# Shamir-Lab/Faucet

Measured on AMD Instinct MI355X. Metric: canonical k-mers/s (load+scan) at k=31, 100bp reads; % HBM roofline, higher is better.
Workload: dtype u64

## Files before the change

### faucet_amd/csrc/api.hip

```cpp
#include <cstdio>
#include <algorithm>
#include <string>

#include <chrono>
#include <thread>

#include "fgpu_ctx.h"

int fgpu_scan_export_impl(fgpu_ctx* ctx, void* dev_entries, uint64_t cap_entries, uint64_t* d_stamps, uint64_t* n_entries);
int fgpu_scan_import_impl(fgpu_ctx* ctx, const void* dev_entries, uint64_t n);
int fgpu_scan_download_impl(fgpu_ctx* ctx, uint64_t* keys_host, fgpu_junction* recs_host, uint64_t cap, uint64_t* n_out);

static thread_local std::string g_create_error;

int g_fgpu_trace = getenv("FGPU_TRACE") && getenv("FGPU_TRACE")[0] == '1';

int fgpu_ensure(fgpu_ctx* ctx, DevBuf* b, uint64_t bytes) {
    if (b->bytes >= bytes && b->p) return FGPU_OK;
    if (b->p) {
        FGPU_HIP(fgpu_sync_stream(ctx, ctx->stream));
        FGPU_HIP(hipFree(b->p));
        b->p = nullptr;
        b->bytes = 0;
    } else {
// ... 604 lines not shown
    if (nbytes) *nbytes = ctx->bloom_bytes;
    return FGPU_OK;
}

int fgpu_bitmap_or(fgpu_ctx* ctx, void* dst_dev, const void* src_dev, uint64_t nbytes) {
    if (!ctx || !dst_dev || !src_dev || (nbytes & 15)) return FGPU_ERR_ARG;
    return fgpu_util_or(ctx, dst_dev, src_dev, nbytes);
}

int fgpu_scan_resident_base(fgpu_ctx* ctx, uint64_t first_batch) {
    if (!ctx) return FGPU_ERR_ARG;
    if (ctx->phase != 0) { ctx->err = "scan_resident_base while a pass is open: between the load pass and fgpu_scan_begin"; return FGPU_ERR_STATE; }
    ctx->scan_resident_base = first_batch;
    return FGPU_OK;
}

int fgpu_scan_begin(fgpu_ctx* ctx) {
    if (!ctx) return FGPU_ERR_ARG;
    if (ctx->phase != 0) { ctx->err = "scan_begin while another pass is open"; return FGPU_ERR_STATE; }
    FGPU_HIP(hipSetDevice(ctx->prm.device));
    int rc = fgpu_bg_join(ctx);
    if (rc) return rc;
    if ((rc = fgpu_scan_alloc(ctx))) return rc;
    if ((rc = fgpu_scan_reset(ctx))) return rc;
    ctx->fixup_ready = false;
    FGPU_HIP(hipMemsetAsync(ctx->counters, 0, sizeof(DevCounters), ctx->stream));
    memset(&ctx->scan_stats, 0, sizeof(ctx->scan_stats));
    memset(ctx->counters_host, 0, sizeof(DevCounters));
    ctx->scan_windows = 0;
    ctx->scan_pieces_seen = 0;
    ctx->scan_piece_base = 0;
    ctx->scan_imported = 0;
    ctx->delta_next = 0;
    journal_recycle(ctx);
    ctx->journal_on = !(ctx->prm.flags & FGPU_FLAG_EAGER_FLAGS) && !ctx->eager_runtime;
    ctx->eager_scan = ctx->lazy_failed = ctx->capacity_failed = false;
    ctx->dl_keys_n = 0;
    ctx->late_acc[0] = ctx->late_acc[1] = ctx->late_acc[2] = 0;
    ctx->stops_delivered = 0;
    ctx->lp_applied_seq = 0;
    ctx->host_waits = 0;
    ctx->host_wait_ms = 0;
    ctx->wait_sites.clear();
    if (ctx->short_pf) FGPU_HIP(hipMemsetAsync(ctx->short_pf, 0, ctx->short_pf_tai / 8, ctx->stream));
    if ((rc = fgpu_long_pairs_reset(ctx))) return rc;
    ctx->have_import = false;
// ... 811 lines not shown
```

### faucet_amd/csrc/fgpu_ctx.h

```cpp
#pragma once
#include <chrono>
#include <hip/hip_runtime.h>
#include <stdint.h>
#include <stdio.h>
#include <string.h>

#include <string>
#include <thread>
#include <vector>

#include "../../include/faucet_gpu.h"
#include <deque>

#include "fgpu_device.h"

#define FGPU_PADW 8
#define FGPU_USUAL_SPAN (1ULL << 26)
#define FGPU_MAX_SPAN (1ULL << 26)

#define FGPU_RANGE_EVENTS 16
#define FGPU_RANGE_MIN (1ULL << 20)

struct DevBuf {
    void*    p = nullptr;
// ... 258 lines not shown
    uint32_t walk_heavy = 0;
    uint32_t* cl_members = nullptr;
    uint32_t* cl_roots = nullptr;
    void* wdesc = nullptr;
    uint64_t window_span = 1ULL << 17;
    uint64_t max_span = FGPU_MAX_SPAN;
    uint64_t settled_span = 0;
    uint64_t scan_piece_base = 0;
    uint64_t scan_imported = 0;
    bool hint_in_table = false;
    uint32_t hint_gen = 0;
    uint64_t hint_n = 0, hint_max_seq = 0;
    uint64_t hint_digest[2] = {0, 0};
    DevBuf delta_filter;
    uint64_t delta_filter_bits = 0;
    bool delta_ready = false;
    uint64_t delta_keys = 0;
    uint64_t refresh_full = 0, refresh_delta = 0, refresh_mismatch = 0;
    DevBuf cand_filter;
    uint64_t sparse_links = 0, full_links = 0;
    int dbg_stall_us = 0;
    bool dbg_delta_check = false;
    bool no_sparse_link = false;
    int scan_range_log2 = -1;
    DevBuf import_probe;
    uint64_t scan_grown = 0;

    DevCounters* counters = nullptr;
    DevCounters* counters_host = nullptr;

    fgpu_load_stats load_stats;
    uint64_t load_mark_hits = 0, load_mark_pending = 0;
    fgpu_scan_stats scan_stats;
    uint64_t scan_windows = 0;
    uint64_t scan_pieces_seen = 0;

    uint64_t adapt_followers = 0, adapt_pieces = 0;
    double host_ms[8] = {0, 0, 0, 0, 0, 0, 0, 0};
    bool repeats_seen_before = false;
    uint64_t calib_ovf = 0;
    uint64_t span_ceiling = ~0ULL;
    int adapt_vote = 0;
    uint64_t proven_span = 0;
    uint64_t adapt_overflows = 0;
    int calib_left = 0;
    uint64_t calib_f = 0, calib_p = 0;
// ... 154 lines not shown
int fgpu_resident_adopt(fgpu_ctx* ctx, const PackedBlock& b);
void fgpu_adopted_release(fgpu_ctx* ctx, std::vector<void*>* blocks);
int fgpu_stage_pack_keep(fgpu_ctx* ctx, const fgpu_reads* reads, uint64_t budget_left, PackedBlock* out, bool* no_memory);
void fgpu_estimate_drop_kept(fgpu_ctx* ctx);
int fgpu_load_sweep(fgpu_ctx* ctx);
int fgpu_stage_fixup(fgpu_ctx* ctx, const uint32_t* prefix);
int fgpu_stage_presence(fgpu_ctx* ctx);
int fgpu_epoch_before_batch(fgpu_ctx* ctx, uint64_t span);
int fgpu_epoch_after_batch(fgpu_ctx* ctx, uint64_t span);
enum { FGPU_TAKE_OK = 0, FGPU_TAKE_NO_BUDGET, FGPU_TAKE_NO_MEMORY };
int fgpu_resident_take(fgpu_ctx* ctx, const uint64_t (&parts)[5], bool budgeted, ResidentBatch** out, uint64_t* total);
int fgpu_pull_counters(fgpu_ctx* ctx);
int fgpu_check_reads(fgpu_ctx* ctx, const fgpu_reads* r);
void fgpu_load_pass_policy(fgpu_ctx* ctx);
int fgpu_load_pass_counters(fgpu_ctx* ctx);
int fgpu_load_pass_end(fgpu_ctx* ctx, fgpu_load_stats* stats);
int fgpu_load_pair_begin(fgpu_ctx* ctx);
int fgpu_load_pair_end(fgpu_ctx* ctx);
void fgpu_resident_reset(fgpu_ctx* ctx, bool keep_going);
int fgpu_stage_scan_pure(fgpu_ctx* ctx, uint64_t* n_pieces, bool one_range);
bool fgpu_walk_no_overlap();
int fgpu_stage_scan_walk(fgpu_ctx* ctx, uint64_t n_pieces);
int fgpu_stage_scan_need(fgpu_ctx* ctx);
int fgpu_stage_scan_need_lookup(fgpu_ctx* ctx, uint64_t w_lo, uint64_t w_hi);
int fgpu_stage_scan_need_prewalk(fgpu_ctx* ctx, uint64_t w_lo, uint64_t w_hi);
int fgpu_scan_refresh_planes(fgpu_ctx* ctx, BatchBufs* b);
int fgpu_scan_build_cand(fgpu_ctx* ctx, BatchBufs* b);
int fgpu_scan_import_probe(fgpu_ctx* ctx, const void* dev_entries, uint64_t n, uint64_t after_seq, uint32_t* dfilter, uint64_t dfilter_bits,
                           uint64_t* max_seq, uint64_t* n_newer, uint64_t digest[2]);
int fgpu_stage_scan_debug_drop(fgpu_ctx* ctx, uint64_t w_lo, uint64_t w_hi);
int fgpu_estimate_range_counts(fgpu_ctx* ctx, uint64_t g0, uint64_t g1, uint64_t h[2 * FGPU_EST_LEVELS + 1]);
void fgpu_estimate_close(fgpu_ctx* ctx, void** later);
int fgpu_estimate_finish(fgpu_ctx* ctx, fgpu_estimate* e, const char* who);
int fgpu_util_count_segments(fgpu_ctx* ctx, const void* bad, uint64_t n_words, int minlen);
int fgpu_util_popcount(fgpu_ctx* ctx, const void* dev, uint64_t nbytes, unsigned long long* dev_out);
int fgpu_util_or(fgpu_ctx* ctx, void* dst, const void* src, uint64_t nbytes);
int fgpu_util_probe_hash(fgpu_ctx* ctx, const uint64_t* d_kmers, uint64_t n, uint64_t* d_canon, uint64_t* d_hA, uint64_t* d_hB);
int fgpu_util_probe_contains(fgpu_ctx* ctx, const uint32_t* bloom, const uint64_t* d_canon, uint64_t n, unsigned char* d_out);
int fgpu_util_probe_stage3(fgpu_ctx* ctx, const uint64_t* d_kmers, uint64_t n, int mode, signed char* d_out);
int fgpu_scan_alloc(fgpu_ctx* ctx);
int fgpu_scan_harvest(fgpu_ctx* ctx, BatchBufs* b);
int fgpu_long_pairs_batch(fgpu_ctx* ctx, const fgpu_stop* d_stops, uint64_t n_stops, uint64_t n_reads);
int fgpu_long_pairs_reset(fgpu_ctx* ctx);
int fgpu_long_pairs_close(fgpu_ctx* ctx);
int fgpu_place_pair(fgpu_ctx* ctx);
int fgpu_scan_reset(fgpu_ctx* ctx);
// ... 6 lines not shown
```

### faucet_amd/csrc/scan_pure.hip

```cpp
#include <algorithm>

#include "fgpu_ctx.h"
#include "fgpu_flags.h"

namespace {

__global__ void __launch_bounds__(256) k_scan_same(const uint64_t* __restrict__ codes, const uint64_t* __restrict__ kept_codes, uint64_t n_code_words,
                                                   const uint64_t* __restrict__ bad, const uint64_t* __restrict__ kept_bad, uint64_t n_words,
                                                   uint32_t* same) {
    bool differ = false;
    for (uint64_t i = (uint64_t)blockIdx.x * blockDim.x + threadIdx.x; i < n_code_words; i += (uint64_t)gridDim.x * blockDim.x) {
        differ |= codes[i] != kept_codes[i];
        if (i < n_words) differ |= bad[i] != kept_bad[i];
    }
    if (__ballot(differ) && fd_lane() == 0) *same = 0;
}

__global__ void __launch_bounds__(256) k_scan_valid(const uint64_t* __restrict__ codes, const uint64_t* __restrict__ bad,
                                                    uint64_t T, uint64_t n_words, FdParams fp, const uint32_t* __restrict__ bloom,
                                                    const uint64_t* __restrict__ sure, const uint32_t* __restrict__ same,
                                                    uint64_t* __restrict__ valid, DevCounters* cnt) {
    unsigned long long n_ok = 0, n_reused = 0;
    const uint64_t total = n_words * 64;
    const bool reuse = sure && *same != 0;
    for (uint64_t p = (uint64_t)blockIdx.x * blockDim.x + threadIdx.x; p < total; p += (uint64_t)gridDim.x * blockDim.x) {
        bool ok = p < T && fd_window_ok(bad, p, fp.k);
        bool v = false;
        if (ok) {
            n_ok++;
            if (reuse && ((sure[p >> 6] >> (p & 63)) & 1ULL)) {
                v = true;
                n_reused++;
            } else {
                v = fd_bloom_contains_canon(bloom, fd_canon(fd_kmer_at(codes, p, fp.k), fp.k), fp.tai_mask, fp.n_hash);
            }
        }
        uint64_t vm = __ballot(v);
        if (fd_lane() == 0) valid[p >> 6] = vm;
    }
    block_add(&cnt->kmers, n_ok);
    block_add(&cnt->valid_reused, n_reused);
}

__global__ void __launch_bounds__(256) k_scan_pieces(const uint64_t* __restrict__ valid, const uint64_t* __restrict__ bad,
                                                     uint64_t n_words, FdParams fp, int check_segment,
                                                     unsigned long long* pm, uint64_t* __restrict__ ps, DevCounters* cnt) {
    unsigned long long n_pieces = 0;
    for (uint64_t w = (uint64_t)blockIdx.x * blockDim.x + threadIdx.x; w < n_words; w += (uint64_t)gridDim.x * blockDim.x) {
        uint64_t vw = valid[w];
        uint64_t prev = w ? valid[w - 1] >> 63 : 0;
        uint64_t starts = vw & ~((vw << 1) | prev);
        uint64_t psw = 0;
        while (starts) {
            const int sbit = __builtin_ctzll(starts);
            starts &= starts - 1;
            const uint64_t p = w * 64 + sbit;
            uint64_t q = p, len = 0;
            for (;;) {
                uint64_t bits = ~fd_bits_at(valid, q);
                if (bits) { len += __builtin_ctzll(bits); break; }
                len += 64;
                q += 64;
            }
            bool piece = len >= (uint64_t)fp.k;
            if (piece && check_segment) {
                uint64_t b = p;
                while (b > 0 && !((bad[(b - 1) >> 6] >> ((b - 1) & 63)) & 1ULL)) b--;
                uint64_t e = p;
                for (;;) {
                    uint64_t bits = fd_bits_at(bad, e);
                    if (bits) { e += __builtin_ctzll(bits); break; }
// ... 443 lines not shown
    int rc;
    uint64_t first, further;
    scan_range_plan(ctx, bb, one_range, &first, &further);
    const uint64_t first_words = std::max<uint64_t>(first / 64, 1), further_words = std::max<uint64_t>(further / 64, 1);
    const uint64_t reach_words = (bb.max_piece_span + 63) / 64 + 1;
    bb.range_first = first_words * 64;
    bb.range_span = further_words * 64;
    bb.n_ranges = bb.n_words <= first_words ? 1 : 1 + (bb.n_words - first_words + further_words - 1) / further_words;
    uint64_t looked = 0;
    for (uint64_t r = 0, lo = 0; lo < bb.n_words; r++) {
        const uint64_t hi = std::min(bb.n_words, lo + (r ? further_words : first_words));
        const uint64_t look_to = std::min(bb.n_words, hi + reach_words);
        if (looked < look_to) {
            if ((rc = fgpu_stage_scan_need_lookup(ctx, looked, look_to))) return rc;
            looked = look_to;
        }
        if ((rc = fgpu_stage_scan_need_prewalk(ctx, lo, hi)) || (rc = scan_pure_flags(ctx, lo, hi)) || (rc = fgpu_stage_scan_debug_drop(ctx, lo, hi))) return rc;
        if (bb.n_ranges > 1) FGPU_HIP(hipEventRecord(bb.range_ev[r % FGPU_RANGE_EVENTS], ctx->stream));
        lo = hi;
    }
    return FGPU_OK;
}

int fgpu_stage_scan_pure(fgpu_ctx* ctx, uint64_t* n_pieces, bool one_range) {
    BatchBufs& bb = *ctx->cur;
    *n_pieces = 0;
    bb.n_pieces = 0;
    bb.n_ranges = 0;
    if (bb.T == 0) return FGPU_OK;
    const uint64_t wb = (bb.n_words + FGPU_PADW) * 8;
    int rc;
    DevBuf* planes[] = {&bb.valid, &bb.pm, &bb.ps, &bb.ff, &bb.fb, &bb.cf0, &bb.cf1, &bb.cb0, &bb.cb1, &bb.inF, &bb.inB, &bb.lk, &bb.nF, &bb.nB, &bb.need};
    for (DevBuf* b : planes)
        if ((rc = fgpu_ensure_b(ctx, b, wb))) return rc;
    if ((rc = fgpu_ensure_b(ctx, &bb.ps_prefix, (bb.n_words + FGPU_PADW + bb.n_words / SCAN_BLOCK + 2) * 4))) return rc;
    const double t_a = fgpu_host_now();
    FGPU_HIP(hipMemsetAsync(bb.valid.p, 0, wb, ctx->stream));
    FGPU_HIP(hipMemsetAsync(bb.pm.p, 0, wb, ctx->stream));
    FGPU_HIP(hipMemsetAsync(bb.ps.p, 0, wb, ctx->stream));

    const unsigned grid = fgpu_grid(bb.n_words * 64, 256);
    const unsigned wgrid = fgpu_grid(bb.n_words, 256);
    if ((rc = fgpu_util_count_segments(ctx, ctx->cur->bad.p, ctx->cur->n_words, ctx->fd.k + 2 * ctx->fd.j + 1))) return rc;
    const uint64_t kept_index = ctx->scan_resident_base + ctx->scan_batch_index;
    const ResidentBatch* kept = kept_index < ctx->resident_count ? ctx->resident[kept_index] : nullptr;
    ctx->scan_batch_index++;
    if (kept && (kept->T != bb.T || kept->n_words != bb.n_words)) kept = nullptr;
    if (kept) {
        if ((rc = fgpu_ensure_b(ctx, &bb.same, 64))) return rc;
        FGPU_HIP(hipMemsetAsync(bb.same.p, 0x01, 4, ctx->stream));
        const uint64_t ncw = 2 * bb.n_words;
        FGPU_LAUNCH("scan_same", k_scan_same, fgpu_grid(ncw, 256), 256, (const uint64_t*)bb.codes.p, (const uint64_t*)kept->codes_p(), ncw,
                    (const uint64_t*)bb.bad.p, (const uint64_t*)kept->bad_p(), bb.n_words, (uint32_t*)bb.same.p);
    }
    FGPU_LAUNCH("scan_valid", k_scan_valid, grid, 256, (const uint64_t*)bb.codes.p, (const uint64_t*)bb.bad.p, bb.T, bb.n_words, ctx->fd,
                (const uint32_t*)ctx->bloo2, kept ? (const uint64_t*)kept->sure.p : (const uint64_t*)nullptr,
                kept ? (const uint32_t*)bb.same.p : (const uint32_t*)nullptr, (uint64_t*)bb.valid.p, ctx->counters);
    const int check_segment = ctx->fd.k < 2 * ctx->fd.j + 2;
    FGPU_LAUNCH("scan_pieces", k_scan_pieces, wgrid, 256, (const uint64_t*)bb.valid.p, (const uint64_t*)bb.bad.p, bb.n_words, ctx->fd,
                check_segment, (unsigned long long*)bb.pm.p, (uint64_t*)bb.ps.p, ctx->counters);
    uint32_t* prefix = (uint32_t*)bb.ps_prefix.p;
    uint32_t* block_sums = prefix + bb.n_words + FGPU_PADW;
    const uint32_t nblk = fgpu_blocks(bb.n_words + 1, SCAN_BLOCK);
    const uint64_t nw1 = bb.n_words + 1;
    FGPU_LAUNCH("prefix_block", k_prefix_block, nblk, SCAN_BLOCK, (const uint64_t*)bb.ps.p, nw1, prefix, block_sums);
    FGPU_LAUNCH("prefix_sums", k_prefix_sums, 1, SCAN_BLOCK, block_sums, nblk);
    FGPU_LAUNCH("prefix_apply", k_prefix_apply, fgpu_blocks(nw1, 256), 256, prefix, (const uint32_t*)block_sums, nw1);
    FGPU_HIP(hipMemcpyAsync(ctx->counters_host, ctx->counters, sizeof(DevCounters), hipMemcpyDeviceToHost, ctx->stream));
    const double t_b = fgpu_host_now();
    FGPU_HIP(fgpu_sync_stream(ctx, ctx->stream));
    const double t_c = fgpu_host_now();
    ctx->host_ms[2] += t_b - t_a;
    ctx->host_ms[3] += t_c - t_b;
    bb.max_piece_span = ctx->counters_host->max_read_len + 64;
    const uint64_t np = ctx->counters_host->pieces - ctx->scan_pieces_seen;
    ctx->scan_pieces_seen = ctx->counters_host->pieces;
    *n_pieces = np;
    bb.n_pieces = np;
    if ((rc = fgpu_ensure_b(ctx, &bb.pieces, (np + 1) * sizeof(uint2)))) return rc;
    if (np) {
        FGPU_LAUNCH("piece_list", k_scan_piece_list, wgrid, 256, (const uint64_t*)bb.ps.p, (const uint64_t*)bb.pm.p,
                    (const uint32_t*)prefix, bb.n_words, (uint2*)bb.pieces.p);
        if (ctx->record_stops) {
            if ((rc = fgpu_ensure_b(ctx, &bb.piece_read, np * 4))) return rc;
            FGPU_LAUNCH("piece_read", k_scan_piece_read, fgpu_blocks(np, 256), 256, (const uint2*)bb.pieces.p, np, bb.d_offs, bb.n_reads,
                        (uint32_t*)bb.piece_read.p);
        }
        if ((rc = fgpu_stage_scan_need(ctx))) return rc;
        DevBuf* outs[] = {&bb.ff, &bb.fb, &bb.cf0, &bb.cf1, &bb.cb0, &bb.cb1};
        for (DevBuf* o : outs) FGPU_HIP(hipMemsetAsync(o->p, 0, wb, ctx->stream));
        if ((rc = scan_pure_back(ctx, one_range))) return rc;
    }
    ctx->host_ms[4] += fgpu_host_now() - t_c;
    return FGPU_OK;
}
```

### faucet_amd/csrc/scan_table.hip

```cpp
#include <algorithm>

#include "walk_tables.h"

#include <rocprim/rocprim.hpp>

namespace {

__global__ void __launch_bounds__(256) k_export(JTable jt, FdParams fp, ExportEntry* out, uint64_t* stamps_out, unsigned long long* n_out) {
    __shared__ unsigned wave_total[4];
    __shared__ unsigned long long block_base;
    const uint64_t n_slots = jt.mask + 1;
    const uint64_t per_block = ((n_slots + gridDim.x - 1) / gridDim.x + 255) & ~255ULL;
    const uint64_t lo = (uint64_t)blockIdx.x * per_block;
    const uint64_t hi = lo + per_block < n_slots ? lo + per_block : n_slots;
    const int wave = (int)(threadIdx.x >> 6);
    unsigned long long mine = 0;
    for (uint64_t s = lo + threadIdx.x; s < hi; s += 256) {
        const uint64_t w = jt.keys[s];
        if (w != J_EMPTY) mine += ((w >> 62) & 1ULL) + ((w >> 63) & 1ULL);
    }
    for (int o = 32; o > 0; o >>= 1) mine += __shfl_down(mine, o, 64);
    if (fd_lane() == 0) wave_total[wave] = (unsigned)mine;
    __syncthreads();
    if (threadIdx.x == 0) {
// ... 141 lines not shown
}

int fgpu_scan_import_probe(fgpu_ctx* ctx, const void* dev_entries, uint64_t n, uint64_t after_seq, uint32_t* dfilter, uint64_t dfilter_bits,
                           uint64_t* max_seq, uint64_t* n_newer, uint64_t digest[2]) {
    *max_seq = *n_newer = 0;
    digest[0] = digest[1] = 0;
    if (!n) return FGPU_OK;
    if (int rc = fgpu_ensure(ctx, &ctx->import_probe, 32)) return rc;
    FGPU_HIP(hipMemsetAsync(ctx->import_probe.p, 0, 32, ctx->stream));
    FGPU_LAUNCH("import", k_import_probe, (unsigned)std::min<uint64_t>(fgpu_blocks(n, 256), 4096), 256, (const ExportEntry*)dev_entries, n, ctx->fd, after_seq, dfilter,
                dfilter_bits ? dfilter_bits - 1 : 0, (unsigned long long*)ctx->import_probe.p);
    unsigned long long out[4] = {0, 0, 0, 0};
    FGPU_HIP(hipMemcpyAsync(out, ctx->import_probe.p, 32, hipMemcpyDeviceToHost, ctx->stream));
    FGPU_HIP(fgpu_sync_stream(ctx, ctx->stream));
    *max_seq = out[0];
    *n_newer = out[1];
    digest[0] = out[2];
    digest[1] = out[3];
    return FGPU_OK;
}

int fgpu_scan_clear_table(fgpu_ctx* ctx) {
    FGPU_HIP(hipMemsetAsync(ctx->jkeys, 0xFF, ctx->jcap * 8, ctx->stream));
    FGPU_HIP(hipMemsetAsync(ctx->jrecs, 0, ctx->jcap * 32, ctx->stream));
    FGPU_HIP(hipMemsetAsync(ctx->jfilter, 0, ctx->jcap * 2 / 8, ctx->stream));
    return FGPU_OK;
}

static int jt_replace_arrays(fgpu_ctx* ctx, uint64_t new_cap, const char* no_memory) {
    uint64_t* nk = nullptr; uint8_t* nr = nullptr; uint64_t* ns = nullptr; uint32_t* nf = nullptr;
    if (hipMalloc(&nk, new_cap * 8) != hipSuccess || hipMalloc(&nr, new_cap * 32) != hipSuccess || hipMalloc(&ns, new_cap * 16) != hipSuccess ||
        hipMalloc(&nf, new_cap * 2 / 8) != hipSuccess) {
        (void)hipGetLastError();
        hipFree(nk); hipFree(nr); hipFree(ns); hipFree(nf);
        ctx->err = no_memory + std::to_string(new_cap) + " slots";
        return FGPU_ERR_NOMEM;
    }
    hipFree(ctx->jkeys); hipFree(ctx->jrecs); hipFree(ctx->jstamps); hipFree(ctx->jfilter);
    ctx->jkeys = nk; ctx->jrecs = nr; ctx->jstamps = ns; ctx->jfilter = nf;
    ctx->jcap = new_cap;
    return FGPU_OK;
}

int fgpu_scan_grow(fgpu_ctx* ctx, uint64_t new_cap) {
    if (new_cap <= ctx->jcap) return FGPU_OK;
    if (ctx->wstream) FGPU_HIP(fgpu_sync_stream(ctx, ctx->wstream));
    FGPU_HIP(fgpu_sync_stream(ctx, ctx->stream));
    FGPU_HIP(hipMemcpyAsync(&ctx->counters_host->n_junctions, &ctx->counters->n_junctions, 8, hipMemcpyDeviceToHost, ctx->stream));
// ... 110 lines not shown
```

### faucet_amd/csrc/scan_walk.hip

```cpp
#include <cstring>
#include <algorithm>

#include "fgpu_flags.h"
#include "walk_tables.h"

namespace {

__device__ __forceinline__ uint32_t uf_find(uint32_t* parent, uint32_t x) {
    uint32_t p = ld_agent(&parent[x]);
    while (p != x) {
        uint32_t gp = ld_agent(&parent[p]);
        if (gp != p) atomicMin(&parent[x], gp);
        x = p;
        p = gp;
    }
    return x;
}

__device__ __forceinline__ void uf_union(uint32_t* parent, uint32_t a, uint32_t b) {
    for (;;) {
        a = uf_find(parent, a);
        b = uf_find(parent, b);
        if (a == b) return;
        if (a < b) { uint32_t t = a; a = b; b = t; }
// ... 639 lines not shown
        KO_T0();
        out.addr = (uint64_t*)(wc.jt.recs + (known_slot * 2 + orient) * 16);
        out.lo = ld_agent(&out.addr[0]);
        out.hi = ld_agent(&out.addr[1]);
        wc.created_now = false;
        if (out.lo == 0xFFFFFFFFFFFFFFF1ULL) return false;
        KO_T1(wc.cnt, 3);
        return true;
    }
    const uint64_t home = fd_mix(canon) & wc.jt.mask;
    const uint64_t* spec = (const uint64_t*)(wc.jt.recs + (home * 2 + orient) * 16);
    const uint64_t w_first = ld_agent(&wc.jt.keys[home]);
    const uint64_t spec_lo = MODE == WALK_KO ? ld_agent(&spec[0]) : spec[0], spec_hi = MODE == WALK_KO ? ld_agent(&spec[1]) : spec[1];
    if (!jt_find_or_claim(wc.jt, canon, home, w_first, slot, present, wc.cnt)) {
        atomicOr(&wc.cnt->error_flags, 1ULL);
        return false;
    }
    out.addr = (uint64_t*)(wc.jt.recs + (slot * 2 + orient) * 16);
    wc.created_now = false;
    if (!((present >> orient) & 1u)) {
        wc.created_now = true;
        atomicOr(&wc.pl.cr[pos >> 6], 1ULL << (pos & 63));
        out.lo = out.hi = 0;
        if (MODE == WALK_KO) st_agent(&wc.jt.stamps[slot * 2 + orient], stamp);
        else wc.jt.stamps[slot * 2 + orient] = stamp;
        atomicOr((unsigned long long*)&wc.jt.keys[slot], 1ULL << (62 + orient));
        const uint64_t hb = jt_filter_bit(wc.jt, canon);
        atomicOr(&wc.jt.filter[hb >> 5], 1u << (hb & 31));
        wc.n_created++;
    } else if (slot == home) {
        out.lo = spec_lo;
        out.hi = spec_hi;
    } else {
        out.lo = MODE == WALK_KO ? ld_agent(&out.addr[0]) : out.addr[0];
        out.hi = MODE == WALK_KO ? ld_agent(&out.addr[1]) : out.addr[1];
    }
    return true;
}


__device__ __forceinline__ bool junction_find(const WalkCtx& wc, uint64_t key, RecRegs& out) {
    const uint64_t rc = fd_revcomp(key, wc.fp.k);
    const uint64_t canon = key < rc ? key : rc;
    const int orient = key == canon ? 0 : 1;
    uint64_t slot;
    uint32_t present;
// ... 893 lines not shown
    const uint4 r = ovw_live_bits(wc.pl.codes, wc.fp.k, v.p0 + 64 * c, where, wc.jt.keys, wc.jt.mask, ow.have_prev ? &ow.prev : nullptr, ow.time);
    mF = (uint64_t)r.x | ((uint64_t)r.y << 32);
    mB = (uint64_t)r.z | ((uint64_t)r.w << 32);
}
__device__ __forceinline__ void ovw_mark_created(const WalkCtx& wc, PieceView& v, uint64_t key) {
    const int k = wc.fp.k;
    for (uint32_t c = 0; c < 2; c++) {
        uint64_t w = c == 0 ? v.lk0 : v.lk1;
        while (w) {
            const uint32_t b = (uint32_t)__builtin_ctzll(w);
            w &= w - 1;
            const uint64_t km = pv_kmer(v, wc.pl.codes, v.p0 + 64 * c + b, k);
            if (km == key) { if (c == 0) v.xF0 |= 1ULL << b; else v.xF1 |= 1ULL << b; }
            if (fd_revcomp(km, k) == key) { if (c == 0) v.xB0 |= 1ULL << b; else v.xB1 |= 1ULL << b; }
        }
    }
}

struct OvwRec {
    uint32_t rec;
    uint64_t lo;
    bool present;
};
__device__ __forceinline__ bool ovw_record(WalkCtx& wc, uint64_t key, OvwRec& out) {
    const uint64_t rc = fd_revcomp(key, wc.fp.k);
    const uint64_t canon = key < rc ? key : rc;
    const int orient = key == canon ? 0 : 1;
    const uint64_t home = fd_mix(canon) & wc.jt.mask;
    const uint64_t* spec = (const uint64_t*)(wc.jt.recs + (home * 2 + orient) * 16);
    const uint64_t w_first = ld_agent(&wc.jt.keys[home]);
    const uint64_t spec_lo = spec[0];
    uint64_t slot;
    uint32_t present;
    if (!jt_find_or_claim(wc.jt, canon, home, w_first, slot, present, wc.cnt)) return false;
    out.rec = (uint32_t)(slot * 2 + orient);
    out.present = (present >> orient) & 1u;
    out.lo = !out.present ? 0ULL : slot == home ? spec_lo : ((const uint64_t*)(wc.jt.recs + (slot * 2 + orient) * 16))[0];
    return true;
}

__device__ __forceinline__ void ovw_walk_piece(WalkCtx& wc, OvwWalk& ow, uint64_t p0, uint32_t nwin) {
    const int k = wc.fp.k, j = wc.fp.j;
    const int tmax = 2 * (int)nwin - 2 - 2 * j;
    const int spacer = 2 * wc.fp.max_spacer - 1;
    PieceView v;
    pv_load(v, wc.pl, p0, nwin);
// ... 70 lines not shown
        const int ext_fwd = fwd ? real : 4, ext_bwd = fwd ? 4 : real;
        OvwRec r;
        {
            const uint32_t at = ow.n_new + (have_last ? 1u : 0u);
            const uint4 o = ow.have_old && at < ow.n_old ? ow.log[at] : make_uint4(0, 0xFFFFFFFFu, 0, 0);
            if ((o.y & 0xFFFF) == (uint32_t)tn && !((o.y >> 16) & OVW_F_FAKE)) {
                r.rec = o.x;
                r.present = ((o.y >> 16) & OVW_F_PRESENT) != 0;
                r.lo = (uint64_t)o.w | ((uint64_t)((o.z >> 8) & 0xFF) << 32);
            } else if (!ovw_record(wc, key, r)) { wc.fail = 1; return; }
        }
        const bool revisit = ovw_seen_test_and_set(r.rec);
        last_pos = tn;
        const uint32_t d_in = (uint32_t)((have_last ? tn - last_t : tn - 2 * j) & 0xFF);
        if (have_last) {
            pend.y |= (OVW_F_LINK_F | OVW_F_DF) << 16;
            pend.z = (pend.z & ~0xFFu) | d_in;
            if (d_in > ((last_lo >> (8 * last_ext_fwd)) & 0xFF) && !ovw_post(ow.cur, pend.x, (uint32_t)last_ext_fwd, ow.time, d_in)) { wc.fail = 1; return; }
            ovw_emit(ow, pend);
        }
        const bool created = !r.present && !(ow.have_prev && ovw_before(ow.prev, r.rec, OVW_CREATION, ow.time)) && !(revisit && ovw_own_created(ow, r.rec));
        uint32_t flags = (created ? OVW_F_CREATED : 0u) | ((uint32_t)real << 1) | (have_last ? OVW_F_LINK_B : 0u) | (r.present ? OVW_F_PRESENT : 0u);
        pend = ovw_pack(r.rec, (uint32_t)tn, flags, d_in, 0, r.lo);
        if (created && !ovw_post(ow.cur, r.rec, OVW_CREATION, ow.time, 1)) { wc.fail = 1; return; }
        if (d_in > ((r.lo >> (8 * ext_bwd)) & 0xFF) && !ovw_post(ow.cur, r.rec, (uint32_t)ext_bwd, ow.time, d_in)) { wc.fail = 1; return; }
        if (created) ovw_mark_created(wc, v, key);
        uint32_t d = (uint32_t)((r.lo >> (8 * ext_fwd)) & 0xFF);
        if (ow.have_prev) d = max(d, ovw_before(ow.prev, r.rec, (uint32_t)ext_fwd, ow.time));
        if (revisit) d = max(d, ovw_own(ow, r.rec, (uint32_t)ext_fwd, pend, true));
        have_last = true;
        last_lo = r.lo;
        last_t = tn;
        last_ext_fwd = ext_fwd;
        if (d < 1) d = 1;
        t = tn + (int)d;
        wc.nb_processed += 1;
        wc.nb_skipped += (unsigned long long)(d - 1);
        if (ow.overflow) { wc.fail = 1; return; }
    }

    if (!have_last) {
        wc.nb_no_juncs++;
        const int len = (int)nwin + k - 1;
        const int m = len / 2 - k / 2;
        const uint64_t key = pv_kmer(v, wc.pl.codes, p0 + m, k);
        const int real = pv_base(v, wc.pl.codes, p0 + m + k);
        const int tm = 2 * m + 1;
        OvwRec r;
        if (!ovw_record(wc, key, r)) { wc.fail = 1; return; }
        const bool created = !r.present && !(ow.have_prev && ovw_before(ow.prev, r.rec, OVW_CREATION, ow.time));
        const uint32_t d_b = (uint32_t)((tm - 2 * j) & 0xFF), d_f = (uint32_t)(((2 * (int)nwin - 1 - tm) - 2 * j) & 0xFF);
        if (created && !ovw_post(ow.cur, r.rec, OVW_CREATION, ow.time, 1)) { wc.fail = 1; return; }
        if (d_b > ((r.lo >> 32) & 0xFF) && !ovw_post(ow.cur, r.rec, 4u, ow.time, d_b)) { wc.fail = 1; return; }
        if (d_f > ((r.lo >> (8 * real)) & 0xFF) && !ovw_post(ow.cur, r.rec, (uint32_t)real, ow.time, d_f)) { wc.fail = 1; return; }
        uint4 e = ovw_pack(r.rec, (uint32_t)tm, (created ? OVW_F_CREATED : 0u) | ((uint32_t)real << 1) | OVW_F_FAKE | OVW_F_DF | (r.present ? OVW_F_PRESENT : 0u), d_b, d_f, r.lo);
        ovw_emit(ow, e);
    } else {
        const uint32_t d_f = (uint32_t)(((2 * (int)nwin - 1 - last_t) - 2 * j) & 0xFF);
        pend.y |= OVW_F_DF << 16;
        pend.z = (pend.z & ~0xFFu) | d_f;
        if (d_f > ((last_lo >> (8 * last_ext_fwd)) & 0xFF) && !ovw_post(ow.cur, pend.x, (uint32_t)last_ext_fwd, ow.time, d_f)) { wc.fail = 1; return; }
        ovw_emit(ow, pend);
    }
    if (ow.overflow) wc.fail = 1;
    if (ow.have_old)
        for (uint32_t i = ow.n_new; i < ow.n_old; i++) {
            const uint4 o = ow.log[i];
            if (ovw_event_sig(o)) ovw_mark(ow, o);
        }
}

__global__ void __launch_bounds__(256) k_ovw_reset(uint32_t* state, uint32_t* filt, uint32_t filt_words3, uint32_t* longp, uint32_t n_pieces,
                                                   uint32_t* marks, uint32_t mark_words3) {
    const uint32_t i = blockIdx.x * blockDim.x + threadIdx.x, stride = gridDim.x * blockDim.x;
// ... 481 lines not shown
            return FGPU_ERR_NOMEM;
        }
        ctx->max_span >>= 1;
    }
}

int fgpu_scan_reset(fgpu_ctx* ctx) {
    if (int rc = fgpu_scan_clear_table(ctx)) return rc;
    if (!ctx->wt_epoch) FGPU_HIP(hipMemsetAsync(ctx->wkeys, 0, ctx->wcap * 8, ctx->stream));
    FGPU_HIP(hipMemsetAsync(ctx->wbits, 0, 2 * (1ULL << ctx->wbits_log2) / 8, ctx->stream));
    FGPU_LAUNCH("iota", k_iota_u32, 64, 256, ctx->uf_parent, (uint64_t)ctx->wmax);
    FGPU_LAUNCH("iota", k_iota_u32, 64, 256, ctx->uf_parent + ctx->wmax, (uint64_t)ctx->wmax);
    FGPU_HIP(hipMemsetAsync(ctx->cl_count, 0, 2 * ctx->wmax * 4, ctx->stream));
    FGPU_HIP(hipMemsetAsync(ctx->cl_offset, 0xFF, 2 * ctx->wmax * 4, ctx->stream));
    FGPU_HIP(hipMemsetAsync(ctx->cl_fail, 0, 2 * ctx->wmax * 4, ctx->stream));
    FGPU_HIP(hipMemsetAsync(ctx->ko_hk, 0xFF, (size_t)ctx->ko_hk_cap * 4 * 2, ctx->stream));
    FGPU_HIP(hipMemsetAsync(ctx->ko_hk + 2 * (size_t)ctx->ko_hk_cap, 0, (size_t)ctx->ko_hk_cap * 4, ctx->stream));
    FGPU_HIP(hipMemsetAsync(ctx->ko_piece, 0, (size_t)ctx->wmax * 4 * 2 + 64, ctx->stream));
    return FGPU_OK;
}

int fgpu_stage_scan_need(fgpu_ctx* ctx) {
    BatchBufs& bb = *ctx->cur;
    const uint64_t wb = (bb.n_words + FGPU_PADW) * 8;
    const bool eager = (ctx->prm.flags & FGPU_FLAG_EAGER_FLAGS) || ctx->eager_runtime || ctx->eager_scan;
    FGPU_HIP(hipMemsetAsync(bb.need.p, eager ? 0xFF : 0, wb, ctx->stream));
    if (!bb.n_pieces) return FGPU_OK;
    return fgpu_ensure_b(ctx, &bb.kh, (bb.n_words + FGPU_PADW) * 64 * 4);
}

int fgpu_stage_scan_need_lookup(fgpu_ctx* ctx, uint64_t w_lo, uint64_t w_hi) {
    BatchBufs& bb = *ctx->cur;
    if (!bb.n_pieces || w_lo >= w_hi) return FGPU_OK;
    FGPU_LAUNCH("need_lookup", k_need_lookup, fgpu_grid((w_hi - w_lo) * 64, 256), 256, (const uint64_t*)bb.codes.p, (const uint64_t*)bb.pm.p,
                w_hi, ctx->fd, make_jt(ctx), (uint64_t*)bb.nF.p, (uint64_t*)bb.nB.p, (uint32_t*)bb.kh.p, w_lo);
    return FGPU_OK;
}

int fgpu_stage_scan_need_prewalk(fgpu_ctx* ctx, uint64_t w_lo, uint64_t w_hi) {
    BatchBufs& bb = *ctx->cur;
    const bool eager = (ctx->prm.flags & FGPU_FLAG_EAGER_FLAGS) || ctx->eager_runtime || ctx->eager_scan;
    if (eager || !bb.n_pieces || w_lo >= w_hi) return FGPU_OK;
    static const int need_tight = getenv("FGPU_NEED_TIGHT") ? atoi(getenv("FGPU_NEED_TIGHT")) : 2;
    const uint64_t most = std::min<uint64_t>(bb.n_pieces, (w_hi - w_lo) * 64 / (uint64_t)(ctx->fd.k + 1) + 2);
    FGPU_LAUNCH("need_prewalk", k_need_prewalk, fgpu_grid(most, 256), 256, (const uint64_t*)bb.codes.p, (const uint2*)bb.pieces.p,
                (const uint32_t*)bb.ps_prefix.p, w_lo, w_hi, ctx->fd, make_jt(ctx), (const uint64_t*)bb.nF.p, (const uint64_t*)bb.nB.p,
                (unsigned long long*)bb.need.p, need_tight);
    return FGPU_OK;
}

int fgpu_scan_refresh_planes(fgpu_ctx* ctx, BatchBufs* b) {
    if (!b->n_pieces || !b->T) return FGPU_OK;
    JTable jt = make_jt(ctx);
    ctx->launch_stream = ctx->stream;
    FGPU_LAUNCH("need_lookup", k_refresh_lookup, fgpu_grid(b->n_words * 64, 256), 256, (const uint64_t*)b->codes.p, (const uint64_t*)b->pm.p, b->n_words,
                ctx->fd, jt, (const uint32_t*)jt.filter, jt.filter_mask, (uint64_t*)b->nF.p, (uint64_t*)b->nB.p, (const uint32_t*)b->kh.p, 0, (uint64_t*)nullptr);
    if (b->pure_done) FGPU_HIP(hipEventRecord(b->pure_done, ctx->stream));
    return FGPU_OK;
}

int fgpu_scan_build_cand(fgpu_ctx* ctx, BatchBufs* b) {
    b->cand_gen = 0;
    if (!b->n_pieces || !b->T) return FGPU_OK;
    int rc;
    const uint64_t wb = (b->n_words + FGPU_PADW) * 8;
    if ((rc = fgpu_ensure_b(ctx, &b->cand, wb)) || (rc = fgpu_ensure(ctx, &ctx->cand_filter, (1ULL << CAND_FILTER_LOG2) / 8))) return rc;
    ctx->launch_stream = ctx->stream;
    FGPU_HIP(hipMemsetAsync(ctx->cand_filter.p, 0, (1ULL << CAND_FILTER_LOG2) / 8, ctx->stream));
    FGPU_HIP(hipMemsetAsync(b->cand.p, 0, wb, ctx->stream));
    const unsigned word_blocks = std::min(fgpu_blocks(b->n_words, 256), 2048u), piece_blocks = std::min(fgpu_blocks(b->n_pieces, 256), 2048u);
    FGPU_LAUNCH("cand_plane", k_cand_mark, word_blocks + piece_blocks, 256, (const uint64_t*)b->pm.p, (const uint64_t*)b->nF.p, (const uint64_t*)b->nB.p,
                (const uint64_t*)b->ff.p, (const uint64_t*)b->fb.p, (const uint32_t*)b->kh.p, b->n_words, (const uint2*)b->pieces.p, b->n_pieces, ctx->fd,
                (uint32_t*)ctx->cand_filter.p, word_blocks);
    FGPU_LAUNCH("cand_plane", k_cand_probe, fgpu_grid(b->n_words * 64, 256), 256, (const uint64_t*)b->pm.p, (const uint32_t*)b->kh.p, b->n_words,
                (const uint32_t*)ctx->cand_filter.p, (uint64_t*)b->cand.p);
    if (b->pure_done) FGPU_HIP(hipEventRecord(b->pure_done, ctx->stream));
    b->cand_gen = ctx->hint_gen;
    return FGPU_OK;
}

int fgpu_stage_scan_debug_drop(fgpu_ctx* ctx, uint64_t w_lo, uint64_t w_hi) {
    static const int drop = getenv("FGPU_DEBUG_NEED_DROP") ? atoi(getenv("FGPU_DEBUG_NEED_DROP")) : 0;
    BatchBufs& bb = *ctx->cur;
    if (!drop || !bb.n_pieces || w_lo >= w_hi) return FGPU_OK;
    if (drop == 2 && ((ctx->prm.flags & FGPU_FLAG_EAGER_FLAGS) || ctx->eager_runtime || ctx->eager_scan)) return FGPU_OK;
    FGPU_LAUNCH("debug_need_drop", k_debug_need_drop, fgpu_grid(w_hi - w_lo, 256), 256, w_lo, w_hi, (uint64_t*)bb.ff.p, (uint64_t*)bb.fb.p,
                (uint64_t*)bb.need.p, (uint64_t*)bb.cf0.p, (uint64_t*)bb.cf1.p, (uint64_t*)bb.cb0.p, (uint64_t*)bb.cb1.p, drop,
                (const uint64_t*)bb.pm.p, (const uint32_t*)bb.kh.p);
    return FGPU_OK;
}

static int env_int(const char* name, int absent) { const char* e = getenv(name); return e ? atoi(e) : absent; }
static bool env_is_one(const char* name) { const char* e = getenv(name); return e && e[0] == '1'; }
struct WalkKnobs {
    const int dbg_walk = env_int("FGPU_DEBUG_WALK", 0);
    const bool serial_clean = env_is_one("FGPU_SERIAL_CLEAN");
    const bool no_overlap = env_is_one("FGPU_NO_OVERLAP");
    const bool no_whole_batch = getenv("FGPU_NO_WHOLE_BATCH") != nullptr;
    const unsigned cluster_grid = (unsigned)std::max(1, env_int("FGPU_CLUSTER_GRID", 256));
    const uint64_t refresh_div = (uint64_t)std::max(1, env_int("FGPU_REFRESH_DIV", 4));
    const unsigned delta_per_block = (unsigned)std::max(1, env_int("FGPU_DELTA_PER_BLOCK", 1024));
    const int ko_avg = getenv("FGPU_WALK_KO_AVG") ? std::min(255, std::max(0, env_int("FGPU_WALK_KO_AVG", 0))) : -1;
    const int ko_avg_min = getenv("FGPU_WALK_KO_AVG_MIN") ? std::min(255, std::max(1, env_int("FGPU_WALK_KO_AVG_MIN", 0))) : -1;
    const uint32_t ko_ticket = (uint32_t)std::max(64, env_int("FGPU_KO_TICKET", 64) / 64 * 64);
    const int ovw_followers = env_int("FGPU_OVW_FOLLOWERS", 0);
    const bool ovw_beside = !env_is_one("FGPU_OVW_SERIAL");
    const unsigned walk_dyn_grid = (unsigned)std::max(1, env_int("FGPU_WALK_DYN_GRID", 1024));
    const bool dbg_span = getenv("FGPU_DEBUG_SPAN") != nullptr;
// ... 458 lines not shown
```

Baseline: 6.037 billion.

## Fold scan plane memsets into scan kernels and drop junction record clearing

```diff
diff --git a/faucet_amd/csrc/api.hip b/faucet_amd/csrc/api.hip
--- a/faucet_amd/csrc/api.hip
+++ b/faucet_amd/csrc/api.hip
@@ -650,6 +650,7 @@
     int rc = fgpu_bg_join(ctx);
     if (rc) return rc;
     if ((rc = fgpu_scan_alloc(ctx))) return rc;
+    ctx->debug_poison = getenv("FGPU_DEBUG_POISON") && getenv("FGPU_DEBUG_POISON")[0] == '1';
     if ((rc = fgpu_scan_reset(ctx))) return rc;
     ctx->fixup_ready = false;
     FGPU_HIP(hipMemsetAsync(ctx->counters, 0, sizeof(DevCounters), ctx->stream));
diff --git a/faucet_amd/csrc/fgpu_ctx.h b/faucet_amd/csrc/fgpu_ctx.h
--- a/faucet_amd/csrc/fgpu_ctx.h
+++ b/faucet_amd/csrc/fgpu_ctx.h
@@ -304,6 +304,7 @@
     int dbg_stall_us = 0;
     bool dbg_delta_check = false;
     bool no_sparse_link = false;
+    bool debug_poison = false;
     int scan_range_log2 = -1;
     DevBuf import_probe;
     uint64_t scan_grown = 0;
@@ -504,6 +505,7 @@
 bool fgpu_walk_no_overlap();
 int fgpu_stage_scan_walk(fgpu_ctx* ctx, uint64_t n_pieces);
 int fgpu_stage_scan_need(fgpu_ctx* ctx);
+static inline bool fgpu_scan_eager(const fgpu_ctx* ctx) { return (ctx->prm.flags & FGPU_FLAG_EAGER_FLAGS) || ctx->eager_runtime || ctx->eager_scan; }
 int fgpu_stage_scan_need_lookup(fgpu_ctx* ctx, uint64_t w_lo, uint64_t w_hi);
 int fgpu_stage_scan_need_prewalk(fgpu_ctx* ctx, uint64_t w_lo, uint64_t w_hi);
 int fgpu_scan_refresh_planes(fgpu_ctx* ctx, BatchBufs* b);
diff --git a/faucet_amd/csrc/scan_pure.hip b/faucet_amd/csrc/scan_pure.hip
--- a/faucet_amd/csrc/scan_pure.hip
+++ b/faucet_amd/csrc/scan_pure.hip
@@ -19,9 +19,9 @@
 __global__ void __launch_bounds__(256) k_scan_valid(const uint64_t* __restrict__ codes, const uint64_t* __restrict__ bad,
                                                     uint64_t T, uint64_t n_words, FdParams fp, const uint32_t* __restrict__ bloom,
                                                     const uint64_t* __restrict__ sure, const uint32_t* __restrict__ same,
-                                                    uint64_t* __restrict__ valid, DevCounters* cnt) {
+                                                    uint64_t* __restrict__ valid, uint64_t* __restrict__ pm, DevCounters* cnt) {
     unsigned long long n_ok = 0, n_reused = 0;
-    const uint64_t total = n_words * 64;
+    const uint64_t total = (n_words + FGPU_PADW) * 64;
     const bool reuse = sure && *same != 0;
     for (uint64_t p = (uint64_t)blockIdx.x * blockDim.x + threadIdx.x; p < total; p += (uint64_t)gridDim.x * blockDim.x) {
         bool ok = p < T && fd_window_ok(bad, p, fp.k);
@@ -36,17 +36,26 @@
             }
         }
         uint64_t vm = __ballot(v);
-        if (fd_lane() == 0) valid[p >> 6] = vm;
+        if (fd_lane() == 0) { valid[p >> 6] = vm; pm[p >> 6] = 0; }
     }
     block_add(&cnt->kmers, n_ok);
     block_add(&cnt->valid_reused, n_reused);
 }
 
+struct FlagPlanes {
+    uint64_t *need, *ff, *fb, *cf0, *cf1, *cb0, *cb1;
+};
 __global__ void __launch_bounds__(256) k_scan_pieces(const uint64_t* __restrict__ valid, const uint64_t* __restrict__ bad,
                                                      uint64_t n_words, FdParams fp, int check_segment,
-                                                     unsigned long long* pm, uint64_t* __restrict__ ps, DevCounters* cnt) {
+                                                     unsigned long long* pm, uint64_t* __restrict__ ps, FlagPlanes out, uint64_t need_fill,
+                                                     DevCounters* cnt) {
     unsigned long long n_pieces = 0;
-    for (uint64_t w = (uint64_t)blockIdx.x * blockDim.x + threadIdx.x; w < n_words; w += (uint64_t)gridDim.x * blockDim.x) {
+    for (uint64_t w = (uint64_t)blockIdx.x * blockDim.x + threadIdx.x; w < n_words + FGPU_PADW; w += (uint64_t)gridDim.x * blockDim.x) {
+        out.need[w] = need_fill;
+        out.ff[w] = 0; out.fb[w] = 0;
+        out.cf0[w] = 0; out.cf1[w] = 0;
+        out.cb0[w] = 0; out.cb1[w] = 0;
+        if (w >= n_words) { ps[w] = 0; continue; }
         uint64_t vw = valid[w];
         uint64_t prev = w ? valid[w - 1] >> 63 : 0;
         uint64_t starts = vw & ~((vw << 1) | prev);
@@ -536,6 +545,11 @@
     return FGPU_OK;
 }
 
+static int scan_poison(fgpu_ctx* ctx, DevBuf* b) {
+    if (b->p) FGPU_HIP(hipMemsetAsync(b->p, 0xA5, b->bytes, ctx->stream));
+    return FGPU_OK;
+}
+
 int fgpu_stage_scan_pure(fgpu_ctx* ctx, uint64_t* n_pieces, bool one_range) {
     BatchBufs& bb = *ctx->cur;
     *n_pieces = 0;
@@ -549,9 +563,11 @@
         if ((rc = fgpu_ensure_b(ctx, b, wb))) return rc;
     if ((rc = fgpu_ensure_b(ctx, &bb.ps_prefix, (bb.n_words + FGPU_PADW + bb.n_words / SCAN_BLOCK + 2) * 4))) return rc;
     const double t_a = fgpu_host_now();
-    FGPU_HIP(hipMemsetAsync(bb.valid.p, 0, wb, ctx->stream));
-    FGPU_HIP(hipMemsetAsync(bb.pm.p, 0, wb, ctx->stream));
-    FGPU_HIP(hipMemsetAsync(bb.ps.p, 0, wb, ctx->stream));
+    if (ctx->debug_poison) {
+        for (DevBuf* b : planes)
+            if ((rc = scan_poison(ctx, b))) return rc;
+        if ((rc = scan_poison(ctx, &bb.ps_prefix)) || (rc = scan_poison(ctx, &bb.kh)) || (rc = scan_poison(ctx, &bb.pieces))) return rc;
+    }
 
     const unsigned grid = fgpu_grid(bb.n_words * 64, 256);
     const unsigned wgrid = fgpu_grid(bb.n_words, 256);
@@ -569,10 +585,12 @@
     }
     FGPU_LAUNCH("scan_valid", k_scan_valid, grid, 256, (const uint64_t*)bb.codes.p, (const uint64_t*)bb.bad.p, bb.T, bb.n_words, ctx->fd,
                 (const uint32_t*)ctx->bloo2, kept ? (const uint64_t*)kept->sure.p : (const uint64_t*)nullptr,
-                kept ? (const uint32_t*)bb.same.p : (const uint32_t*)nullptr, (uint64_t*)bb.valid.p, ctx->counters);
+                kept ? (const uint32_t*)bb.same.p : (const uint32_t*)nullptr, (uint64_t*)bb.valid.p, (uint64_t*)bb.pm.p, ctx->counters);
     const int check_segment = ctx->fd.k < 2 * ctx->fd.j + 2;
-    FGPU_LAUNCH("scan_pieces", k_scan_pieces, wgrid, 256, (const uint64_t*)bb.valid.p, (const uint64_t*)bb.bad.p, bb.n_words, ctx->fd,
-                check_segment, (unsigned long long*)bb.pm.p, (uint64_t*)bb.ps.p, ctx->counters);
+    const uint64_t need_fill = fgpu_scan_eager(ctx) ? ~0ULL : 0ULL;
+    const FlagPlanes out{(uint64_t*)bb.need.p, (uint64_t*)bb.ff.p, (uint64_t*)bb.fb.p, (uint64_t*)bb.cf0.p, (uint64_t*)bb.cf1.p, (uint64_t*)bb.cb0.p, (uint64_t*)bb.cb1.p};
+    FGPU_LAUNCH("scan_pieces", k_scan_pieces, fgpu_grid(bb.n_words + FGPU_PADW, 256), 256, (const uint64_t*)bb.valid.p, (const uint64_t*)bb.bad.p, bb.n_words, ctx->fd,
+                check_segment, (unsigned long long*)bb.pm.p, (uint64_t*)bb.ps.p, out, need_fill, ctx->counters);
     uint32_t* prefix = (uint32_t*)bb.ps_prefix.p;
     uint32_t* block_sums = prefix + bb.n_words + FGPU_PADW;
     const uint32_t nblk = fgpu_blocks(bb.n_words + 1, SCAN_BLOCK);
@@ -591,7 +609,9 @@
     ctx->scan_pieces_seen = ctx->counters_host->pieces;
     *n_pieces = np;
     bb.n_pieces = np;
+    const void* const pieces_was = bb.pieces.p;
     if ((rc = fgpu_ensure_b(ctx, &bb.pieces, (np + 1) * sizeof(uint2)))) return rc;
+    if (ctx->debug_poison && bb.pieces.p != pieces_was && (rc = scan_poison(ctx, &bb.pieces))) return rc;
     if (np) {
         FGPU_LAUNCH("piece_list", k_scan_piece_list, wgrid, 256, (const uint64_t*)bb.ps.p, (const uint64_t*)bb.pm.p,
                     (const uint32_t*)prefix, bb.n_words, (uint2*)bb.pieces.p);
@@ -600,9 +620,9 @@
             FGPU_LAUNCH("piece_read", k_scan_piece_read, fgpu_blocks(np, 256), 256, (const uint2*)bb.pieces.p, np, bb.d_offs, bb.n_reads,
                         (uint32_t*)bb.piece_read.p);
         }
+        const void* const kh_was = bb.kh.p;
         if ((rc = fgpu_stage_scan_need(ctx))) return rc;
-        DevBuf* outs[] = {&bb.ff, &bb.fb, &bb.cf0, &bb.cf1, &bb.cb0, &bb.cb1};
-        for (DevBuf* o : outs) FGPU_HIP(hipMemsetAsync(o->p, 0, wb, ctx->stream));
+        if (ctx->debug_poison && bb.kh.p != kh_was && (rc = scan_poison(ctx, &bb.kh))) return rc;
         if ((rc = scan_pure_back(ctx, one_range))) return rc;
     }
     ctx->host_ms[4] += fgpu_host_now() - t_c;
diff --git a/faucet_amd/csrc/scan_table.hip b/faucet_amd/csrc/scan_table.hip
--- a/faucet_amd/csrc/scan_table.hip
+++ b/faucet_amd/csrc/scan_table.hip
@@ -187,8 +187,11 @@
 
 int fgpu_scan_clear_table(fgpu_ctx* ctx) {
     FGPU_HIP(hipMemsetAsync(ctx->jkeys, 0xFF, ctx->jcap * 8, ctx->stream));
-    FGPU_HIP(hipMemsetAsync(ctx->jrecs, 0, ctx->jcap * 32, ctx->stream));
     FGPU_HIP(hipMemsetAsync(ctx->jfilter, 0, ctx->jcap * 2 / 8, ctx->stream));
+    if (ctx->debug_poison) {
+        FGPU_HIP(hipMemsetAsync(ctx->jrecs, 0xA5, ctx->jcap * 32, ctx->stream));
+        FGPU_HIP(hipMemsetAsync(ctx->jstamps, 0xA5, ctx->jcap * 16, ctx->stream));
+    }
     return FGPU_OK;
 }
 
diff --git a/faucet_amd/csrc/scan_walk.hip b/faucet_amd/csrc/scan_walk.hip
--- a/faucet_amd/csrc/scan_walk.hip
+++ b/faucet_amd/csrc/scan_walk.hip
@@ -685,6 +685,7 @@
         wc.created_now = true;
         atomicOr(&wc.pl.cr[pos >> 6], 1ULL << (pos & 63));
         out.lo = out.hi = 0;
+        rr_store_m<MODE>(out);
         if (MODE == WALK_KO) st_agent(&wc.jt.stamps[slot * 2 + orient], stamp);
         else wc.jt.stamps[slot * 2 + orient] = stamp;
         atomicOr((unsigned long long*)&wc.jt.keys[slot], 1ULL << (62 + orient));
@@ -1624,6 +1625,11 @@
     uint64_t lo;
     bool present;
 };
+__device__ __forceinline__ void ovw_zero_record(const WalkCtx& wc, uint32_t rec) {
+    uint64_t* const r = (uint64_t*)(wc.jt.recs + (uint64_t)rec * 16);
+    r[0] = 0;
+    r[1] = 0;
+}
 __device__ __forceinline__ bool ovw_record(WalkCtx& wc, uint64_t key, OvwRec& out) {
     const uint64_t rc = fd_revcomp(key, wc.fp.k);
     const uint64_t canon = key < rc ? key : rc;
@@ -1740,6 +1746,7 @@
         const bool created = !r.present && !(ow.have_prev && ovw_before(ow.prev, r.rec, OVW_CREATION, ow.time)) && !(revisit && ovw_own_created(ow, r.rec));
         uint32_t flags = (created ? OVW_F_CREATED : 0u) | ((uint32_t)real << 1) | (have_last ? OVW_F_LINK_B : 0u) | (r.present ? OVW_F_PRESENT : 0u);
         pend = ovw_pack(r.rec, (uint32_t)tn, flags, d_in, 0, r.lo);
+        if (created) ovw_zero_record(wc, r.rec);
         if (created && !ovw_post(ow.cur, r.rec, OVW_CREATION, ow.time, 1)) { wc.fail = 1; return; }
         if (d_in > ((r.lo >> (8 * ext_bwd)) & 0xFF) && !ovw_post(ow.cur, r.rec, (uint32_t)ext_bwd, ow.time, d_in)) { wc.fail = 1; return; }
         if (created) ovw_mark_created(wc, v, key);
@@ -1768,6 +1775,7 @@
         if (!ovw_record(wc, key, r)) { wc.fail = 1; return; }
         const bool created = !r.present && !(ow.have_prev && ovw_before(ow.prev, r.rec, OVW_CREATION, ow.time));
         const uint32_t d_b = (uint32_t)((tm - 2 * j) & 0xFF), d_f = (uint32_t)(((2 * (int)nwin - 1 - tm) - 2 * j) & 0xFF);
+        if (created) ovw_zero_record(wc, r.rec);
         if (created && !ovw_post(ow.cur, r.rec, OVW_CREATION, ow.time, 1)) { wc.fail = 1; return; }
         if (d_b > ((r.lo >> 32) & 0xFF) && !ovw_post(ow.cur, r.rec, 4u, ow.time, d_b)) { wc.fail = 1; return; }
         if (d_f > ((r.lo >> (8 * real)) & 0xFF) && !ovw_post(ow.cur, r.rec, (uint32_t)real, ow.time, d_f)) { wc.fail = 1; return; }
@@ -2295,9 +2303,6 @@
 
 int fgpu_stage_scan_need(fgpu_ctx* ctx) {
     BatchBufs& bb = *ctx->cur;
-    const uint64_t wb = (bb.n_words + FGPU_PADW) * 8;
-    const bool eager = (ctx->prm.flags & FGPU_FLAG_EAGER_FLAGS) || ctx->eager_runtime || ctx->eager_scan;
-    FGPU_HIP(hipMemsetAsync(bb.need.p, eager ? 0xFF : 0, wb, ctx->stream));
     if (!bb.n_pieces) return FGPU_OK;
     return fgpu_ensure_b(ctx, &bb.kh, (bb.n_words + FGPU_PADW) * 64 * 4);
 }
@@ -2312,8 +2317,7 @@
 
 int fgpu_stage_scan_need_prewalk(fgpu_ctx* ctx, uint64_t w_lo, uint64_t w_hi) {
     BatchBufs& bb = *ctx->cur;
-    const bool eager = (ctx->prm.flags & FGPU_FLAG_EAGER_FLAGS) || ctx->eager_runtime || ctx->eager_scan;
-    if (eager || !bb.n_pieces || w_lo >= w_hi) return FGPU_OK;
+    if (fgpu_scan_eager(ctx) || !bb.n_pieces || w_lo >= w_hi) return FGPU_OK;
     static const int need_tight = getenv("FGPU_NEED_TIGHT") ? atoi(getenv("FGPU_NEED_TIGHT")) : 2;
     const uint64_t most = std::min<uint64_t>(bb.n_pieces, (w_hi - w_lo) * 64 / (uint64_t)(ctx->fd.k + 1) + 2);
     FGPU_LAUNCH("need_prewalk", k_need_prewalk, fgpu_grid(most, 256), 256, (const uint64_t*)bb.codes.p, (const uint2*)bb.pieces.p,
@@ -2356,7 +2360,7 @@
     static const int drop = getenv("FGPU_DEBUG_NEED_DROP") ? atoi(getenv("FGPU_DEBUG_NEED_DROP")) : 0;
     BatchBufs& bb = *ctx->cur;
     if (!drop || !bb.n_pieces || w_lo >= w_hi) return FGPU_OK;
-    if (drop == 2 && ((ctx->prm.flags & FGPU_FLAG_EAGER_FLAGS) || ctx->eager_runtime || ctx->eager_scan)) return FGPU_OK;
+    if (drop == 2 && fgpu_scan_eager(ctx)) return FGPU_OK;
     FGPU_LAUNCH("debug_need_drop", k_debug_need_drop, fgpu_grid(w_hi - w_lo, 256), 256, w_lo, w_hi, (uint64_t*)bb.ff.p, (uint64_t*)bb.fb.p,
                 (uint64_t*)bb.need.p, (uint64_t*)bb.cf0.p, (uint64_t*)bb.cf1.p, (uint64_t*)bb.cb0.p, (uint64_t*)bb.cb1.p, drop,
                 (const uint64_t*)bb.pm.p, (const uint32_t*)bb.kh.p);
```

Result: no change. 6.031 billion (-0.1%).
